# sumansamui/CMOOP_Audio_Processing

Hardware: AMD Instinct MI355X
Metric: candidate-net evals/hour (pop=40, GSC-v2) (higher is better)
Workload: dtype f32

## Files before the change

### cmoop_audio_processing_amd/_lib.py

```python
from __future__ import annotations

import ctypes as C
import os
import re
import subprocess
import threading

_HERE = os.path.dirname(os.path.abspath(__file__))
CSRC = os.path.join(_HERE, "csrc")
LIB_PATH = os.environ.get("CMOOP_LIB_PATH") or os.path.join(CSRC, "libcmoop_hip.so")
HEADER = os.path.join(os.path.dirname(_HERE), "include", "cmoop.h")

_lock = threading.Lock()
_lib = None


class CmoopError(RuntimeError):
    pass


class Config(C.Structure):
    _fields_ = [(n, C.c_int32) for n in (
        "variant", "classes", "epochs", "batch", "patience", "early_stop", "restore_best", "acc_readout",
        "fpr_variant", "shuffle", "eval_batch", "n_slots", "profile_every", "gemm_mode")] + \
# ... 355 lines not shown

def plan_convs(gene, variant, T, F):
    g, n, cap = (C.c_int32 * 6)(*gene), C.c_int32(), 16
    rows = (C.c_int32 * (7 * cap))()
    check(lib().cmoop_plan_convs(g, C.c_int32(variant), C.c_int32(T), C.c_int32(F), rows, C.c_int32(cap), C.byref(n)))
    assert n.value <= cap
    return [tuple(rows[7 * i:7 * i + 7]) for i in range(n.value)]


def plan_dwconvs(gene, variant, T, F):
    g, n, cap = (C.c_int32 * 6)(*gene), C.c_int32(), 16
    rows = (C.c_int32 * (4 * cap))()
    check(lib().cmoop_plan_dwconvs(g, C.c_int32(variant), C.c_int32(T), C.c_int32(F), rows, C.c_int32(cap), C.byref(n)))
    assert n.value <= cap
    return [tuple(rows[4 * i:4 * i + 4]) for i in range(n.value)]


def dwconv_wgrad_slices(B, H, W, Cn, KS):
    out = C.c_int32()
    check(lib().cmoop_dwconv_wgrad_slices(B, H, W, Cn, KS, C.byref(out)))
    return int(out.value)


def net_launch_plan(gene, config, T, F, B, train):
    g, buf = (C.c_int32 * 6)(*gene), C.create_string_buffer(8192)
    check(lib().cmoop_net_launch_plan(g, C.byref(config), C.c_int32(T), C.c_int32(F), C.c_int32(B), C.c_int32(int(train)), buf,
                                      C.c_int32(8192)))
    return [k for k in buf.value.decode().split(";") if k]


def profile_entries():
    L, cnt, out = lib(), C.c_int32(), []
    check(L.cmoop_profile_count(C.byref(cnt)))
    for i in range(cnt.value):
        name, n, ms, fl = C.create_string_buffer(160), C.c_int64(), C.c_double(), C.c_double()
        check(L.cmoop_profile_entry(i, name, 160, C.byref(n), C.byref(ms), C.byref(fl)))
        out.append((name.value.decode(), int(n.value), float(ms.value), float(fl.value)))
    return out


def profile_variants():
    L, cnt, out = lib(), C.c_int32(), []
    check(L.cmoop_profile_variant_count(C.byref(cnt)))
    for i in range(cnt.value):
        name = C.create_string_buffer(200)
        check(L.cmoop_profile_variant(i, name, 200))
# ... 13 lines not shown
```

### cmoop_audio_processing_amd/csrc/api.hip

```cpp
#include "../../include/cmoop.h"
#include "net.h"

#include <cstddef>
#include <cstring>
#include <memory>
#include <mutex>
#include <vector>

using namespace cmoop;

static thread_local std::string g_err;
static thread_local std::string g_last_kernels;

template <class F>
static int guard(F&& f) {
    try {
        f();
        return 0;
    } catch (const std::exception& e) {
        g_err = e.what();
        return 1;
    } catch (...) {
        g_err = "unknown error";
        return 2;
// ... 1298 lines not shown
        CMOOP_REQUIRE(out, "dwconv_wgrad_slices: NULL output");
        *out = dwconv_wgrad_slices(B, H, W, C, KS);
    });
}

int cmoop_net_launch_plan(const int32_t gene[6], const cmoop_config* cfg, int32_t T, int32_t F, int32_t B, int32_t train, char* buf,
                          int32_t cap) {
    return guard([&] {
        CMOOP_REQUIRE(gene && buf && cap > 0 && T >= 1 && F >= 1, "net_launch_plan: bad arguments");
        const NetConfig c = to_cfg(cfg);
        const std::string v = plan_net(gene, c, T, F).launch_plan(c.batch, std::max(c.batch, c.eval_batch), B, train != 0);
        CMOOP_REQUIRE((int)v.size() < cap, "net_launch_plan: buffer too small");
        std::memcpy(buf, v.c_str(), v.size() + 1);
    });
}

int cmoop_halo_tile_check(int32_t B, int32_t H, int32_t W, int32_t Cin, int32_t Cout, int32_t KS, int32_t* rows_bound,
                          int32_t* rows_needed, int32_t* rows_stageable) {
    return guard([&] {
        CMOOP_REQUIRE(rows_bound && rows_needed && rows_stageable && B >= 1 && H >= 1 && W >= 1 && Cin >= 16 && Cout >= 1 && KS >= 1, "bad conv shape");
        int b = 0, n = 0, c = 0;
        halo_rows_bound_and_need(conv_geometry(B, H, W, Cin, Cout, KS, 1), &b, &n, &c);
        *rows_bound = b; *rows_needed = n; *rows_stageable = c;
    });
}

int cmoop_wgrad_slices(int32_t B, int32_t H, int32_t W, int32_t Cin, int32_t Cout, int32_t KS, int32_t stride, int32_t* out) {
    return guard([&] {
        CMOOP_REQUIRE(out && B >= 1 && H >= 1 && W >= 1 && Cin >= 1 && Cout >= 1 && KS >= 1 && stride >= 1, "bad conv shape");
        *out = wgrad_slices(conv_geometry(B, H, W, Cin, Cout, KS, stride));
    });
}

int cmoop_calculate_fpr(const int32_t* y_true, const int32_t* y_pred, int64_t n, int32_t classes, int32_t fpr_variant,
                        double* out) {
    return guard([&] {
        CMOOP_REQUIRE(classes >= 1 && classes <= 4096, "bad class count");
        std::vector<int64_t> cm((size_t)classes * classes, 0);
        for (int64_t i = 0; i < n; ++i) {
            const int a = fpr_variant == CMOOP_FPR_V1_QUIRK ? 0 : y_true[i];
            const int b = y_pred[i];
            if (a >= 0 && a < classes && b >= 0 && b < classes) cm[(size_t)a * classes + b] += 1;
        }
        *out = fpr_from_confusion(cm.data(), classes, fpr_variant == CMOOP_FPR_V3 ? 2 : 0);
    });
}
// ... 759 lines not shown
        CMOOP_HIP(hipStreamSynchronize(s));
    });
}

int cmoop_conv_bwd_trainer(const float* x, const float* w, const float* dy, float* dx, float* dw, float* db, int32_t B, int32_t H,
                           int32_t W, int32_t Cin, int32_t Cout, int32_t KS, int32_t stride, int32_t mask_relu) {
    return guard([&] {
        g_last_kernels.clear();
        hipStream_t s = lib_stream();
        Scratch m(s);
        const ConvLayer L{H, W, Cin, Cout, KS, stride};
        RecordingHook hook(&g_last_kernels);
        const size_t NK = L.flip_floats();
        ConvBuffers buf;
        buf.slab_floats = L.slab_floats_at(B);
        buf.slabs = m.floats(buf.slab_floats);
        float* dwb = m.floats(NK + Cout);
        buf.tab_rows = L.table_rows(B);
        buf.tab = m.rowtab(L.geometry(B), buf.tab_rows);
        L.wgrad(x, dy, dwb, dwb + NK, B, buf, GEMM_DEFAULT, s, &hook);
        CMOOP_HIP(hipMemcpyAsync(dw, dwb, NK * 4, hipMemcpyDeviceToDevice, s));
        CMOOP_HIP(hipMemcpyAsync(db, dwb + NK, (size_t)Cout * 4, hipMemcpyDeviceToDevice, s));
        if (dx) {
            int accumulate = 0;
            if (stride != 1) {
                CMOOP_HIP(hipMemsetAsync(dx, 0, (size_t)B * H * W * Cin * 4, s));
                accumulate = 1;
            }
            if (L.mfma_dgrad()) {
                buf.wd = m.floats(NK);
                launch_flip_transpose(w, buf.wd, Cout, KS, KS, Cin, s);
                buf.tab_d_rows = L.dgrad_table_rows(B);
                buf.tab_d = m.rowtab(L.dgrad_geom(B), buf.tab_d_rows);
                buf.splitk_floats = igemm_splitk_workspace(L.dgrad_geom(B));
                buf.splitk = m.floats(buf.splitk_floats);
            }
            L.dgrad(dy, w, dx, B, mask_relu ? x : nullptr, 1.f, accumulate, L.mfma_dgrad(), buf, GEMM_DEFAULT, s, &hook);
        }
        CMOOP_HIP(hipStreamSynchronize(s));
    });
}

int cmoop_last_kernels(char* buf, int32_t cap) {
    return guard([&] {
        CMOOP_REQUIRE(buf && cap > 0, "last_kernels: no buffer");
        std::snprintf(buf, cap, "%s", g_last_kernels.c_str());
    });
}

int cmoop_conv_time(int32_t mode, const float* x, const float* w, const float* bias, float* y, int32_t B, int32_t H,
                    int32_t W, int32_t Cin, int32_t Cout, int32_t KS, int32_t iters, double* avg_ms) {
    return guard([&] {
        hipStream_t s = lib_stream();
        Scratch m(s);
        const ConvLayer L{H, W, Cin, Cout, KS, 1};
        const ConvGeom g = L.geometry(B), gd = L.dgrad_geom(B);
        float *wd = nullptr, *wg = nullptr;
        GemmEpilogue e;
        const int S = wgrad_slices(g);
        if (mode == 0) e.bias = bias;
// ... 287 lines not shown
```

### cmoop_audio_processing_amd/csrc/gemm.hip

```cpp
#include "kernels.h"
#include <hip/hip_ext.h>
#include <cstdlib>
#include <mutex>
#include <string>
#include <type_traits>

namespace cmoop {

typedef __bf16 bf16x8 __attribute__((ext_vector_type(8)));
typedef unsigned u32x4 __attribute__((ext_vector_type(4)));

typedef __bf16 bf16x2 __attribute__((ext_vector_type(2)));

template <int NP>
__device__ __forceinline__ void split_pair(const float x, const float y, unsigned (&w)[NP]) {
    if constexpr (NP == 1) {
        w[0] = __builtin_bit_cast(unsigned, __builtin_convertvector((f32x2){x, y}, bf16x2));
    } else {
        const unsigned ux = __float_as_uint(x), uy = __float_as_uint(y);
        w[0] = __builtin_amdgcn_perm(uy, ux, 0x07060302u);
        const float rx = x - __uint_as_float(ux & 0xFFFF0000u), ry = y - __uint_as_float(uy & 0xFFFF0000u);
        const unsigned vx = __float_as_uint(rx), vy = __float_as_uint(ry);
        w[1] = __builtin_amdgcn_perm(vy, vx, 0x07060302u);
        const float sx = rx - __uint_as_float(vx & 0xFFFF0000u), sy = ry - __uint_as_float(vy & 0xFFFF0000u);
// ... 7 lines not shown
int gemm_mode_default() {
    static const int v = [] {
        const char* e = std::getenv("CMOOP_GEMM_MODE");
        if (!e) return (int)GEMM_FP32;
        const std::string m(e);
        return m == "bf16x3" ? (int)GEMM_BF16X3 : (m == "bf16" ? (int)GEMM_BF16 : (int)GEMM_FP32);
    }();
    return v;
}
static int resolve_mode(int mode) {
    const int m = mode >= 0 ? mode : gemm_mode_default();
    return (m == GEMM_BF16X3 || m == GEMM_BF16) ? m : GEMM_FP32;
}

struct GeomDev {
    int B, H, W, Cin, OH, OW, Cout, KH, KW, stride, pad_t, pad_l;
    int M, K, cshift, OHW;
    uint32_t ohw_magic, ohw_shift, ow_magic, ow_shift;
    int rcp_kw;
    const float* zeros;
};
struct EpiDev {
    int bal_L, bal_segmax;
    float* stats;
    const float* bias;
    const float* mask;
    float mask_scale;
    int relu, accumulate, out_stride, OHf, OWf, dropout;
    uint32_t drop_prefix, drop_thr;
    float drop_scale;
};

static double par_scale() {
    static const double v = [] {
        const char* e = std::getenv("CMOOP_PAR_SCALE");
        const double x = e ? std::atof(e) : 1.0;
        return x > 0.01 && x <= 4.0 ? x : 1.0;
    }();
    return v;
}

__device__ __forceinline__ int fastdiv(int n, uint32_t magic, uint32_t shift) {
    return (int)((__umulhi((uint32_t)n, magic) + (uint32_t)n) >> shift);
}

static const float* zero_page() {
// ... 575 lines not shown
                red[((wave / WN) * BN + c) * 2 + 1] = csq[ct];
            }
        }
        __syncthreads();
        if (t < BN && n0 + t < N) {
            float a = 0.f, b = 0.f;
#pragma unroll
            for (int w = 0; w < WM; ++w) { a += red[(w * BN + t) * 2]; b += red[(w * BN + t) * 2 + 1]; }
            e.stats[((size_t)mtile * 2) * N + n0 + t] = a;
            e.stats[((size_t)mtile * 2 + 1) * N + n0 + t] = b;
        }
    }
    }
}

struct HaloDev {
    int WP, rows_max, VH;
    uint32_t wp_magic, wp_shift, vh_magic, vh_shift;
};
__host__ __device__ constexpr int halo_nst(int bm) { return bm == 256 ? 11 : 9; }
static bool halo_geometry(const ConvGeom& cg, HaloDev* hd, size_t* lds_bytes);
static size_t halo_balanced_slab_floats(const ConvGeom& cg, int* L_out);

template <int KS, int BM, int BN, int WM, bool BAL = false>
__global__ __launch_bounds__(256, 2) void halo_fwd_kernel(const float* __restrict__ X, const float* __restrict__ Wt,
                                                          float* __restrict__ Y, GeomDev g, EpiDev e, HaloDev h,
                                                          float* __restrict__ slab) {
    constexpr int WN = 4 / WM, RT = BM / WM / 16, CT = BN / WN / 16, R = KS / 2, T = KS * KS;
    constexpr int PITCH = 24;
    constexpr int NST = halo_nst(BM);
    static_assert(RT >= 1 && CT >= 1, "tile too small for the wave layout");
    extern __shared__ __attribute__((aligned(16))) float halo[];

    const int t = threadIdx.x;
    const int ncc = g.Cin >> 4;
    const int upt = ncc * KS;
    int u = 0, uend = 1;
    if constexpr (BAL) {
        const int U = ((g.M + BM - 1) / BM) * ((g.Cout + BN - 1) / BN) * upt;
        u = blockIdx.x * e.bal_L;
        uend = min(U, u + e.bal_L);
    }
    while (u < uend) {
    int mtile, ntile, c_lo = 0, c_hi = upt;
    float* pslab = nullptr;
    if constexpr (BAL) {
        const int nt = (g.Cout + BN - 1) / BN;
        const int t0 = u / upt;
        c_lo = u - t0 * upt;
        c_hi = min(upt, c_lo + (uend - u));
        mtile = t0 / nt; ntile = t0 - mtile * nt;
        const int seg = c_lo == 0 ? 0 : (int)blockIdx.x - (t0 * upt) / e.bal_L;
        pslab = slab + ((size_t)t0 * e.bal_segmax + seg) * (BM * BN);
        u += c_hi - c_lo;
        __syncthreads();
    } else {
        u = uend;
        mtile = blockIdx.x;
        const int nwg = gridDim.x, xcd = mtile & 7, idx = mtile >> 3;
        const int qn = nwg >> 3, rn = nwg & 7;
        mtile = (xcd < rn ? xcd * (qn + 1) : rn * (qn + 1) + (xcd - rn) * qn) + idx;
        ntile = blockIdx.y;
    }
    const int m0 = mtile * BM, n0 = ntile * BN;
    const int wave = t >> 6, lane = t & 63, lr = lane & 15, q = lane >> 4;
    const int wrow = (wave / WN) * (BM / WM), wcol = (wave % WN) * (BN / WN);

    auto vrow = [&](int m, int& x) {
        const int b = fastdiv(m, g.ohw_magic, g.ohw_shift), r = m - b * g.OHW;
        const int y = fastdiv(r, g.ow_magic, g.ow_shift);
        x = r - y * g.OW;
        return b * h.VH + y;
    };
    int xdummy;
    const int vbase = vrow(m0, xdummy);
    const int vlast = vrow(min(m0 + BM, g.M) - 1, xdummy);
    const int items = (vlast - vbase + 1 + 2 * R) * h.WP * 4;

    const __amdgpu_buffer_rsrc_t xr = __builtin_amdgcn_make_buffer_rsrc(
        const_cast<float*>(X), 0, (int)((uint32_t)g.B * g.H * g.W << g.cshift) * 4, 0x00020000);
// ... 82 lines not shown
#pragma unroll
                for (int j = 0; j < 4; ++j)
#pragma unroll
                    for (int rt = 0; rt < RT; ++rt)
#pragma unroll
                        for (int ct = 0; ct < CT; ++ct)
                            acc[rt][ct] = __builtin_amdgcn_mfma_f32_16x16x4f32(ac[rt][j], bc[ct][j], acc[rt][ct], 0, 0, 0);
                __builtin_amdgcn_s_setprio(0);
#pragma unroll
                for (int ct = 0; ct < CT; ++ct) bc[ct] = bn[ct];
                if (kx + 1 < KS || (!last_unit && !new_cc)) {
#pragma unroll
                    for (int rt = 0; rt < RT; ++rt) ac[rt] = an[rt];
                } else if (!last_unit) {
                    __syncthreads();
                    stage_store();
                    __syncthreads();
#pragma unroll
                    for (int rt = 0; rt < RT; ++rt) ac[rt] = *reinterpret_cast<const f32x4*>(a_ptr[rt]);
                }
            }
            ky = nky; cc = ncc2;
        }
#pragma unroll
        for (int rt = 0; rt < RT; ++rt)
#pragma unroll
            for (int r = 0; r < 4; ++r)
#pragma unroll
                for (int ct = 0; ct < CT; ++ct)
                    pslab[(wrow + rt * 16 + q * 4 + r) * BN + wcol + ct * 16 + lr] = acc[rt][ct][r];
        continue;
    } else {
    f32x4 ac[RT], bc[CT];
    stage_load(0);
    load_b(0, 0, bc);
    stage_store();
    __syncthreads();
#pragma unroll
    for (int rt = 0; rt < RT; ++rt) ac[rt] = *reinterpret_cast<const f32x4*>(a_ptr[rt]);

    for (int cc = 0; cc < ncc; ++cc) {
        const bool more = cc + 1 < ncc;
#pragma unroll
        for (int tap = 0; tap < T; ++tap) {
            f32x4 an[RT], bn[CT];
#pragma unroll
            for (int ct = 0; ct < CT; ++ct) bn[ct] = bc[ct];
            if (tap + 1 < T) {
                load_b(cc, tap + 1, bn);
                const int ky = (tap + 1) / KS, kx = (tap + 1) % KS;
#pragma unroll
                for (int rt = 0; rt < RT; ++rt)
                    an[rt] = *reinterpret_cast<const f32x4*>(a_ptr[rt] + ky * wp_f + kx * PITCH);
            } else if (more) {
// ... 7 lines not shown
                for (int rt = 0; rt < RT; ++rt)
#pragma unroll
                    for (int ct = 0; ct < CT; ++ct)
                        acc[rt][ct] = __builtin_amdgcn_mfma_f32_16x16x4f32(ac[rt][j], bc[ct][j], acc[rt][ct], 0, 0, 0);
            __builtin_amdgcn_s_setprio(0);
#pragma unroll
            for (int ct = 0; ct < CT; ++ct) bc[ct] = bn[ct];
            if (tap + 1 < T) {
#pragma unroll
                for (int rt = 0; rt < RT; ++rt) ac[rt] = an[rt];
            } else if (more) {
                __syncthreads();
                stage_store();
                __syncthreads();
#pragma unroll
                for (int rt = 0; rt < RT; ++rt) ac[rt] = *reinterpret_cast<const f32x4*>(a_ptr[rt]);
            }
        }
    }

    }

    const int N = g.Cout;
    float csum[CT], csq[CT], bias_v[CT];
#pragma unroll
    for (int ct = 0; ct < CT; ++ct) {
        csum[ct] = 0.f; csq[ct] = 0.f;
        const int col = n0 + wcol + ct * 16 + lr;
        bias_v[ct] = (e.bias && col < N) ? e.bias[col] : 0.f;
    }
    const bool whole = m0 + BM <= g.M && (N % BN) == 0;
    const uint32_t e_lane = (uint32_t)((m0 + wrow + q * 4) * N + n0 + wcol + lr) * 4u;
    const __amdgpu_buffer_rsrc_t yrs = __builtin_amdgcn_make_buffer_rsrc(Y, 0, g.M * N * 4, 0x00020000);
    if (whole && !e.dropout && !e.mask && !e.accumulate) {
        auto store_all = [&](auto relu_c, auto stats_c) {
#pragma unroll
            for (int rt = 0; rt < RT; ++rt)
#pragma unroll
                for (int r = 0; r < 4; ++r) {
                    const int soff = (rt * 16 + r) * N * 4;
#pragma unroll
                    for (int ct = 0; ct < CT; ++ct) {
                        float v = acc[rt][ct][r] + bias_v[ct];
                        if constexpr (decltype(relu_c)::value) v = fmaxf(v, 0.f);
                        __builtin_amdgcn_raw_buffer_store_b32(__float_as_uint(v), yrs, (int)(e_lane + ct * 64), soff, 0);
                        if constexpr (decltype(stats_c)::value) { csum[ct] += v; csq[ct] += v * v; }
                    }
                }
        };
        using T1 = std::integral_constant<bool, true>;
        using T0 = std::integral_constant<bool, false>;
        if (e.relu) { if (e.stats) store_all(T1{}, T1{}); else store_all(T1{}, T0{}); }
        else        { if (e.stats) store_all(T0{}, T1{}); else store_all(T0{}, T0{}); }
    } else if (whole && e.mask && !e.dropout && !e.relu && !e.bias && !e.stats) {
        const __amdgpu_buffer_rsrc_t mrs = __builtin_amdgcn_make_buffer_rsrc(const_cast<float*>(e.mask), 0, g.M * N * 4, 0x00020000);
#pragma unroll
        for (int rt = 0; rt < RT; ++rt) {
            float mk[4][CT], old[4][CT];
#pragma unroll
            for (int r = 0; r < 4; ++r)
#pragma unroll
                for (int ct = 0; ct < CT; ++ct) {
                    const int soff = (rt * 16 + r) * N * 4;
                    mk[r][ct] = __uint_as_float(__builtin_amdgcn_raw_buffer_load_b32(mrs, (int)(e_lane + ct * 64), soff, 0));
                    old[r][ct] = e.accumulate ? __uint_as_float(__builtin_amdgcn_raw_buffer_load_b32(yrs, (int)(e_lane + ct * 64), soff, 0)) : 0.f;
                }
#pragma unroll
            for (int r = 0; r < 4; ++r)
#pragma unroll
                for (int ct = 0; ct < CT; ++ct) {
                    const int soff = (rt * 16 + r) * N * 4;
                    float v = (mk[r][ct] > 0.f) ? acc[rt][ct][r] * e.mask_scale : 0.f;
                    if (e.accumulate) v += old[r][ct];
                    __builtin_amdgcn_raw_buffer_store_b32(__float_as_uint(v), yrs, (int)(e_lane + ct * 64), soff, 0);
                }
        }
    } else {
// ... 4 lines not shown
            const int row = m0 + wrow + rt * 16 + q * 4 + r;
            if (row >= g.M) continue;
            const size_t rbase = (size_t)row * N;
#pragma unroll
            for (int ct = 0; ct < CT; ++ct) {
                const int col = n0 + wcol + ct * 16 + lr;
                if (col >= N) continue;
                float v = acc[rt][ct][r] + bias_v[ct];
                if (e.relu) v = fmaxf(v, 0.f);
                const size_t off = rbase + col;
                if (e.dropout) {
                    uint32_t u24 = fmix32(e.drop_prefix ^ (uint32_t)((size_t)row * N + col)) >> 8;
                    v = (u24 >= e.drop_thr) ? v * e.drop_scale : 0.f;
                }
                if (e.mask) v = (e.mask[off] > 0.f) ? v * e.mask_scale : 0.f;
                if (e.accumulate) v += Y[off];
                Y[off] = v;
                csum[ct] += v;
                csq[ct] += v * v;
            }
        }
    }
    }
    if (e.stats) {
        __syncthreads();
        float* red = halo;
#pragma unroll
        for (int ct = 0; ct < CT; ++ct) {
            csum[ct] += __shfl_xor(csum[ct], 16, 64);
            csq[ct] += __shfl_xor(csq[ct], 16, 64);
            csum[ct] += __shfl_xor(csum[ct], 32, 64);
            csq[ct] += __shfl_xor(csq[ct], 32, 64);
            if (q == 0) {
                const int c = wcol + ct * 16 + lr;
                red[((wave / WN) * BN + c) * 2] = csum[ct];
                red[((wave / WN) * BN + c) * 2 + 1] = csq[ct];
            }
        }
        __syncthreads();
        if (t < BN && n0 + t < N) {
            float a = 0.f, b = 0.f;
#pragma unroll
            for (int w = 0; w < WM; ++w) { a += red[(w * BN + t) * 2]; b += red[(w * BN + t) * 2 + 1]; }
            e.stats[((size_t)mtile * 2) * N + n0 + t] = a;
            e.stats[((size_t)mtile * 2 + 1) * N + n0 + t] = b;
        }
    }
    }
}

struct BalDev { int bm, bn, nt, chunks, L, segmax; };

template <int VEC>
__global__ __launch_bounds__(256) void splitk_combine_kernel(const float* __restrict__ P, float* __restrict__ Y, GeomDev g,
                                                             EpiDev e, int splits, BalDev bal) {
    const int N = g.Cout;
    const size_t total = (size_t)g.M * N;
    for (size_t i = ((size_t)blockIdx.x * 256 + threadIdx.x) * VEC; i < total; i += (size_t)gridDim.x * 256 * VEC) {
        const int row = (int)(i / N), col = (int)(i - (size_t)row * N);
        float v[VEC];
#pragma unroll
        for (int j = 0; j < VEC; ++j) v[j] = 0.f;
        if (bal.L > 0) {
            const int mt = row / bal.bm, ntl = col / bal.bn;
            const int tile = mt * bal.nt + ntl;
            const int first = (tile * bal.chunks) / bal.L;
            const int nseg = ((tile + 1) * bal.chunks + bal.L - 1) / bal.L - first;
            const float* src = P + (size_t)tile * bal.segmax * (bal.bm * bal.bn) + (size_t)(row - mt * bal.bm) * bal.bn + (col - ntl * bal.bn);
            for (int z = 0; z < nseg; ++z) {
                if constexpr (VEC == 4) {
                    const f32x4 p = *reinterpret_cast<const f32x4*>(src + (size_t)z * (bal.bm * bal.bn));
                    v[0] += p[0]; v[1] += p[1]; v[2] += p[2]; v[3] += p[3];
                } else {
                    v[0] += src[(size_t)z * (bal.bm * bal.bn)];
                }
            }
        } else
        for (int z = 0; z < splits; ++z) {
            if constexpr (VEC == 4) {
                const f32x4 p = *reinterpret_cast<const f32x4*>(P + (size_t)z * total + i);
                v[0] += p[0]; v[1] += p[1]; v[2] += p[2]; v[3] += p[3];
            } else {
                v[0] += P[(size_t)z * total + i];
            }
        }
        size_t off = i;
        if (e.out_stride != 1) {
            int b = fastdiv(row, g.ohw_magic, g.ohw_shift), rr = row - b * g.OHW;
            int oh = fastdiv(rr, g.ow_magic, g.ow_shift), ow = rr - oh * g.OW;
            off = ((size_t)(b * e.OHf + oh * e.out_stride) * e.OWf + ow * e.out_stride) * N + col;
        }
#pragma unroll
        for (int j = 0; j < VEC; ++j) {
            float x = v[j];
            if (e.bias) x += e.bias[col + j];
            if (e.relu) x = fmaxf(x, 0.f);
            if (e.dropout) {
                uint32_t u24 = fmix32(e.drop_prefix ^ (uint32_t)(i + j)) >> 8;
                x = (u24 >= e.drop_thr) ? x * e.drop_scale : 0.f;
            }
            if (e.mask) x = (e.mask[off + j] > 0.f) ? x * e.mask_scale : 0.f;
            if (e.accumulate) x += Y[off + j];
            v[j] = x;
        }
        if constexpr (VEC == 4) *reinterpret_cast<f32x4*>(Y + off) = f32x4{v[0], v[1], v[2], v[3]};
        else Y[off] = v[0];
    }
// ... 110 lines not shown
    *bm = 64; *bn = bn_small;
}

size_t igemm_splitk_workspace(const ConvGeom& g) {
    const int M = g.M(), N = g.Cout;
    const int bn_big = N > 64 ? 128 : (N <= 16 ? 16 : (N <= 32 ? 32 : 64));
    const long blocks = (long)cdiv(M, 128) * cdiv(N, bn_big);
    if (blocks >= 384) return 0;
    const int sp = std::min(32, cdiv(1024, (int)blocks));
    return std::max(std::max((size_t)sp * M * N, balanced_slab_floats(M, N, g.K(), g.Cin % 32 == 0 ? 32 : 16, bn_big, nullptr)),
                    halo_balanced_slab_floats(g, nullptr));
}

static size_t halo_balanced_slab_floats(const ConvGeom& cg, int* L_out) {
    static const bool on = [] { const char* v = std::getenv("CMOOP_HALO_BAL"); return !(v && v[0] == '0'); }();
    if (!on || cg.Cout % 64 != 0 || !halo_geometry(cg, nullptr, nullptr)) return 0;
    const long tiles = (long)cdiv(cg.M(), 128) * (cg.Cout / 64);
    const int upt = (cg.Cin / 16) * cg.KH;
    const long units = tiles * upt;
    if (tiles >= 1024 || units < 512l * 2 * cg.KH) return 0;
    const int L = (int)((units + 511) / 512);
    if (L_out) *L_out = L;
    return (size_t)tiles * (cdiv(upt, L) + 1) * 128 * 64;
}

struct FwdChoice {
    int mode, bm, bn, splits, balanced_wgs, flags;
    bool bk32_tile, use_dma, stats, halo;
    int ks, halo_L;
    int code() const { return mode * 100000000 + bm * 100000 + bn * 100 + (halo ? ks + (halo_L > 0 ? 50 : 0) : (bk32_tile ? 32 : 16)); }
};

static inline int halo_bm(int cout) { return cout >= 64 ? 128 : 256; }
static bool halo_geometry(const ConvGeom& cg, HaloDev* hd, size_t* lds_bytes) {
    const int ks = cg.KH, R = ks / 2;
    if (cg.KH != cg.KW || (ks != 3 && ks != 5) || cg.stride != 1 || cg.OH != cg.H || cg.OW != cg.W) return false;
    if (cg.pad_t != R || cg.pad_l != R || cg.Cin % 16 != 0) return false;
    if (cg.Cout % 64 != 0 && cg.Cout != 32 && cg.Cout != 16) return false;
    const int bm = halo_bm(cg.Cout);
    const int wp = (cg.W + ks - 1 + 7) / 8 * 8;
    const int span = (bm - 2 + cg.W) / cg.W + 1 + ((bm - 1) / (cg.H * cg.W) + 1) * R;
    const int rows = span + 2 * R;
    if (rows * wp * 4 > halo_nst(bm) * 256) return false;
    const size_t lds = (size_t)rows * wp * 24 * sizeof(float);
    if (lds > 64 * 1024) return false;
    if (hd) {
// ... 47 lines not shown
        c.bm = halo_bm(cg.Cout);
        c.bn = std::min(cg.Cout, 64);
    } else if (halo_env && (c.mode == GEMM_FP32 || c.mode == GEMM_FP32_DMA) && c.bm == 128 && (c.splits > 1 || c.balanced_wgs) && ep.out_stride == 1) {
        int L = 0;
        const size_t need = halo_balanced_slab_floats(cg, &L);
        if (need > 0 && need <= ws_floats) {
            c.halo = true; c.halo_L = L; c.mode = GEMM_FP32_HALO; c.use_dma = false; c.stats = false;
            c.bm = 128; c.bn = 64; c.splits = 1; c.balanced_wgs = 512;
        }
    }
    c.flags = (c.splits > 1 ? GEMM_FLAG_SPLITK : 0) | (c.stats ? GEMM_FLAG_STATS : 0) | (c.balanced_wgs ? GEMM_FLAG_BALANCED : 0) |
              ((!c.halo && have_rowtab && (cg.Cin % bk) == 0 && cg.KH * cg.KW <= 32) ? GEMM_FLAG_ROWTAB : 0);
    return c;
}

int igemm_fwd_plan(const ConvGeom& g, const GemmEpilogue& ep, size_t ws_floats, bool want_stats, bool have_rowtab, int* flags_out) {
    igemm_check_range(g);
    CMOOP_REQUIRE(ilog2_exact(g.Cin) >= 4, "implicit GEMM needs C_in a power of two >= 16");
    const FwdChoice c = choose_fwd(g, ep, ws_floats, want_stats, have_rowtab);
    if (flags_out) *flags_out = c.flags;
    return c.code();
}

int launch_igemm_fwd(const float* X, const float* Wt, float* Y, const ConvGeom& cg, const GemmEpilogue& ep,
                     hipStream_t s, const GemmTiming* tm, float* splitk_ws, size_t splitk_ws_floats, int* stats_blocks,
                     const void* rowtab_v, int tab_rows, int* flags_out) {
    if (stats_blocks) *stats_blocks = 0;
    if (flags_out) *flags_out = 0;
    const uint2* rowtab = static_cast<const uint2*>(rowtab_v);
    GeomDev g = to_dev(cg);
    if (g.M == 0) return 0;
    EpiDev e;
    e.bias = ep.bias; e.mask = ep.mask; e.mask_scale = ep.mask_scale; e.relu = ep.relu;
    e.accumulate = ep.accumulate; e.out_stride = ep.out_stride; e.OHf = ep.OHf; e.OWf = ep.OWf;
    e.dropout = ep.dropout; e.drop_prefix = ep.drop_prefix; e.drop_thr = ep.drop_thr; e.drop_scale = ep.drop_scale;
    if (e.out_stride > 1)
        CMOOP_REQUIRE((int64_t)g.B * e.OHf * e.OWf * g.Cout < (1ll << 29), "scattered output too large");
    const FwdChoice ch = choose_fwd(cg, ep, splitk_ws ? splitk_ws_floats : 0, ep.stats != nullptr && stats_blocks != nullptr, rowtab != nullptr);
    const int mode = ch.mode == GEMM_FP32_DMA ? (int)GEMM_FP32 : ch.mode;
    const int bm = ch.bm, bn = ch.bn, splits = ch.splits, balanced_wgs = ch.balanced_wgs;
    const bool bk32_tile = ch.bk32_tile, use_dma = ch.use_dma;
    e.bal_L = 0; e.bal_segmax = 0;
    e.stats = ch.stats ? ep.stats : nullptr;
    if (e.stats) *stats_blocks = cdiv(g.M, bm);
    if (flags_out) *flags_out = ch.flags;
    if (ch.halo) {
        HaloDev hd;
        size_t lds = 0;
        CMOOP_REQUIRE(halo_geometry(cg, &hd, &lds), "halo kernel chosen for a geometry it does not accept");
        dim3 grid(cdiv(g.M, bm), cdiv(g.Cout, bn));
        BalDev bal{bm, bn, cdiv(g.Cout, bn), (cg.Cin / 16) * cg.KH, ch.halo_L, 0};
        if (ch.halo_L > 0) {
            bal.segmax = cdiv(bal.chunks, bal.L) + 1;
            e.bal_L = bal.L; e.bal_segmax = bal.segmax;
            const long units = (long)grid.x * grid.y * bal.chunks;
            grid = dim3((unsigned)((units + bal.L - 1) / bal.L), 1, 1);
            lds = std::max(lds, (size_t)55 * 1024);
        }
        static const int occ_env = [] { const char* v = std::getenv("CMOOP_HALO_OCC"); const int o = v ? std::atoi(v) : 0; return o == 2 || o == 3 ? o : 0; }();
        lds = halo_lds_for_occupancy(lds, (long)grid.x * grid.y, occ_env);
        auto run = [&](auto kernel) { launch_timed(kernel, grid, lds, s, tm, X, Wt, Y, g, e, hd, splitk_ws); };
#define CMOOP_HALO_KS(KS_)                                                                     \
        do {                                                                                   \
            if (ch.halo_L > 0) run(halo_fwd_kernel<KS_, 128, 64, 2, true>);                    \
            else if (bn == 64) run(halo_fwd_kernel<KS_, 128, 64, 2, false>);                   \
            else if (bn == 32) run(halo_fwd_kernel<KS_, 256, 32, 4, false>);                   \
            else run(halo_fwd_kernel<KS_, 256, 16, 4, false>);                                 \
        } while (0)
        if (cg.KH == 5) CMOOP_HALO_KS(5); else CMOOP_HALO_KS(3);
#undef CMOOP_HALO_KS
        CMOOP_HIP(hipGetLastError());
        if (ch.halo_L > 0) {
            const size_t total = (size_t)g.M * g.Cout;
            const unsigned gridc = (unsigned)std::min<size_t>((total / 4 + 255) / 256, 4096);
            hipLaunchKernelGGL(splitk_combine_kernel<4>, dim3(gridc), dim3(256), 0, s, splitk_ws, Y, g, e, 2, bal);
            CMOOP_HIP(hipGetLastError());
        }
        return ch.code();
    }
#define CMOOP_FWD(BM_, BN_, WM_)                                                              \
    do {                                                                                      \
        if (mode == GEMM_BF16X3) launch_fwd_t<BM_, BN_, 32, WM_, GEMM_BF16X3>(X, Wt, Y, g, e, s, tm, splitk_ws, splits, balanced_wgs, rowtab, tab_rows);   \
        else if (mode == GEMM_BF16) launch_fwd_t<BM_, BN_, 32, WM_, GEMM_BF16>(X, Wt, Y, g, e, s, tm, splitk_ws, splits, balanced_wgs, rowtab, tab_rows);  \
        else if (use_dma && BM_ == 128 && BN_ == 32) launch_fwd_t<BM_, 32, 32, WM_, GEMM_FP32_DMA>(X, Wt, Y, g, e, s, tm, splitk_ws, splits, balanced_wgs, rowtab, tab_rows);   \
        else if (bk32_tile) launch_fwd_t<BM_, BN_, 32, WM_>(X, Wt, Y, g, e, s, tm, splitk_ws, splits, balanced_wgs, rowtab, tab_rows);   \
        else launch_fwd_t<BM_, BN_, 16, WM_>(X, Wt, Y, g, e, s, tm, splitk_ws, splits, 0, rowtab, tab_rows);        \
    } while (0)
    if (bm == 128) {
        if (bn == 128) CMOOP_FWD(128, 128, 2);
        else if (bn == 64) CMOOP_FWD(128, 64, 4);
        else if (bn == 32) CMOOP_FWD(128, 32, 4);
        else CMOOP_FWD(128, 16, 4);
    } else {
        if (bn == 64) CMOOP_FWD(64, 64, 2);
        else if (bn == 32) CMOOP_FWD(64, 32, 4);
        else CMOOP_FWD(64, 16, 4);
// ... 796 lines not shown
```

### cmoop_audio_processing_amd/csrc/kernels.h

```cpp
#pragma once
#include "common.h"
#include <string>
#include <vector>

namespace cmoop {

struct ConvGeom {
    int B, H, W, Cin;
    int OH, OW, Cout;
    int KH, KW, stride;
    int pad_t, pad_l;
    int M() const { return B * OH * OW; }
    int K() const { return KH * KW * Cin; }
};
inline ConvGeom conv_geometry(int B, int H, int W, int Cin, int Cout, int KS, int stride) {
    ConvGeom g;
    g.B = B; g.H = H; g.W = W; g.Cin = Cin; g.Cout = Cout; g.KH = g.KW = KS; g.stride = stride;
    g.OH = (H + stride - 1) / stride; g.OW = (W + stride - 1) / stride;
    const int th = (g.OH - 1) * stride + KS - H, tw = (g.OW - 1) * stride + KS - W;
    g.pad_t = (th > 0 ? th : 0) / 2; g.pad_l = (tw > 0 ? tw : 0) / 2;
    return g;
}

enum GemmMode { GEMM_DEFAULT = -1, GEMM_FP32 = 0, GEMM_FP32_DMA = 1 , GEMM_BF16X3 = 2, GEMM_BF16 = 3,
// ... 8 lines not shown
    float mask_scale = 1.f;
    int accumulate = 0;
    int out_stride = 1;
    int OHf = 0, OWf = 0;
    int dropout = 0;
    uint32_t drop_prefix = 0, drop_thr = 0;
    float drop_scale = 1.f;
    float* stats = nullptr;
};

struct GemmTiming {
    hipEvent_t start = nullptr, stop = nullptr;
    bool ext = true;
};
enum GemmFlags { GEMM_FLAG_SPLITK = 1, GEMM_FLAG_STATS = 2, GEMM_FLAG_ROWTAB = 4, GEMM_FLAG_BALANCED = 8, GEMM_FLAG_SLABS = 16 };
int launch_igemm_fwd(const float* X, const float* Wt, float* Y, const ConvGeom& g,
                     const GemmEpilogue& e, hipStream_t s, const GemmTiming* tm = nullptr,
                     float* splitk_ws = nullptr, size_t splitk_ws_floats = 0, int* stats_blocks = nullptr,
                     const void* rowtab = nullptr, int tab_rows = 0, int* flags_out = nullptr);
size_t igemm_splitk_workspace(const ConvGeom& g);
int igemm_fwd_plan(const ConvGeom& g, const GemmEpilogue& e, size_t ws_floats, bool want_stats, bool have_rowtab, int* flags_out);
int igemm_wgrad_plan(const ConvGeom& g, int S, int mode, bool have_rowtab, int* flags_out);
void halo_rows_bound_and_need(const ConvGeom& g, int* bound, int* need, int* items_cap);
void igemm_check_range(const ConvGeom& g);
std::string gemm_kernel_name(int cls, int code);

int wgrad_slices(const ConvGeom& g);
int launch_igemm_wgrad(const float* X, const float* dY, float* P, const ConvGeom& g, int S, hipStream_t s,
                       const GemmTiming* tm = nullptr, float* Pbias = nullptr, size_t slab_stride = 0,
                       int mode = GEMM_DEFAULT, const void* rowtab = nullptr, int tab_rows = 0, int* flags_out = nullptr);
int rowtab_rows(const ConvGeom& g);
void launch_build_rowtab(const ConvGeom& g, void* tab, hipStream_t s);
void launch_reduce_slices(const float* P, float* out, int S, int64_t n, hipStream_t s, int64_t stride = 0);
void launch_flip_transpose(const float* W, float* Wd, int Cout, int KH, int KW, int Cin, hipStream_t s);
struct FlipEntry { int64_t w_off, wd_off; int Cout, KH, KW, Cin; };
void launch_flip_transpose_all(const float* params, float* wd_all, const FlipEntry* table_dev, int layers, int64_t max_elems,
                               hipStream_t s);

struct StepState {
    long long row0;
    unsigned step;
    unsigned iter;
};
void launch_step_advance(StepState* st, int batch, hipStream_t s);
struct BatchRows {
    const int32_t* idx = nullptr;
// ... 404 lines not shown
```

### include/cmoop.h

```cpp
#ifndef CMOOP_H
#define CMOOP_H

#include <stdint.h>

#ifdef __cplusplus
extern "C" {
#endif

#define CMOOP_ABI_VERSION 3

#define CMOOP_VARIANT_A 0
#define CMOOP_VARIANT_B 1
#define CMOOP_VARIANT_A_DS 2
#define CMOOP_VARIANT_B_DS 3

#define CMOOP_FPR_V1 0
#define CMOOP_FPR_V1_QUIRK 1
#define CMOOP_FPR_V3 2

#define CMOOP_GEMM_DEFAULT 0
#define CMOOP_GEMM_FP32 1
#define CMOOP_GEMM_BF16X3 2
#define CMOOP_GEMM_BF16 3

// ... 278 lines not shown
                             const cmoop_optim* optim, const cmoop_ema* ema, const cmoop_opoint* op, const cmoop_quant* q,
                             const cmoop_prune* pr, const cmoop_actquant* aq, const cmoop_dataset* ds, const int32_t* genes ,
                             const uint32_t* seeds , int32_t n, cmoop_next_fn next, void* ctx, double* acc, double* size_mb,
                             double* fpr, int32_t* epochs_run, double* val_loss, double* seconds, int32_t* evaluated,
                             double* opoint , double* quant ,
                             double* prune );

int cmoop_plan_check(const int32_t gene[6], int32_t variant, int32_t T, int32_t F, int32_t batch);

int cmoop_conv_launch_plan(int32_t op, int32_t B, int32_t H, int32_t W, int32_t Cin, int32_t Cout, int32_t KS, int32_t stride,
                           int32_t want_stats, char* name, int32_t name_cap);

int cmoop_plan_convs(const int32_t gene[6], int32_t variant, int32_t T, int32_t F, int32_t* layers , int32_t cap,
                     int32_t* count);

int cmoop_plan_dwconvs(const int32_t gene[6], int32_t variant, int32_t T, int32_t F, int32_t* layers , int32_t cap,
                       int32_t* count);

int cmoop_net_launch_plan(const int32_t gene[6], const cmoop_config* cfg, int32_t T, int32_t F, int32_t B, int32_t train,
                          char* buf, int32_t cap);

int cmoop_halo_tile_check(int32_t B, int32_t H, int32_t W, int32_t Cin, int32_t Cout, int32_t KS, int32_t* rows_bound,
                          int32_t* rows_needed, int32_t* rows_stageable);

int cmoop_wgrad_slices(int32_t B, int32_t H, int32_t W, int32_t Cin, int32_t Cout, int32_t KS, int32_t stride, int32_t* out);

int cmoop_dwconv_wgrad_slices(int32_t B, int32_t H, int32_t W, int32_t C, int32_t KS, int32_t* out);

int cmoop_calculate_fpr(const int32_t* y_true, const int32_t* y_pred, int64_t n, int32_t classes, int32_t fpr_variant,
                        double* out);

int cmoop_logmel(const float* wav_dev , int64_t n_clips, int32_t n_samples,
                 float* out_dev );
typedef struct cmoop_frontend_config {
    int32_t sr, n_fft, win, hop, n_mels;
    int32_t scale;
    int32_t db_ref_max;
    float fmin, fmax, log_eps, db_amin, top_db;
} cmoop_frontend_config;
int cmoop_frontend_config_default(cmoop_frontend_config* c);
int cmoop_frontend_check(const cmoop_frontend_config* c);
int cmoop_frontend_frames(const cmoop_frontend_config* c, int32_t n_samples, int32_t* T);
int cmoop_frontend_mel_basis(const cmoop_frontend_config* c, float* out_host);
int cmoop_logmel_ex(const cmoop_frontend_config* c, const float* wav_dev , int64_t n_clips,
                    int32_t n_samples, float* out_dev );
int cmoop_logmel_ex_time(const cmoop_frontend_config* c, const float* wav_dev, int64_t n_clips, int32_t n_samples, float* out_dev,
// ... 174 lines not shown
```

Baseline: 440.9.

## Give each balanced halo workgroup one whole tile plus a stream-K share

Restructures the stream-K balanced halo forward conv so that each of the G workgroups first computes one complete output tile through the normal epilogue, then splits the remaining tiles' K-units evenly. Only the split tiles go through the slab workspace and the combine kernel. This cuts slab writes and combine traffic for most of the output. It is gated on an env switch (on by default) and on workspace fitting, and the combine kernel gains a tile-indexed path. A host-side partition checker is added for validation, and the dgrad test entry gains an accumulate flag.

```diff
diff --git a/cmoop_audio_processing_amd/_lib.py b/cmoop_audio_processing_amd/_lib.py
--- a/cmoop_audio_processing_amd/_lib.py
+++ b/cmoop_audio_processing_amd/_lib.py
@@ -401,6 +401,22 @@
     return int(out.value)
 
 
+HALO_BAL_FIELDS = ("T", "upt", "L", "G", "s", "whole", "slab_floats", "workgroups", "most_units", "finished_in_kernel", "cut_tiles",
+                   "slab_pieces", "units_not_owned_once", "slab_faults", "combine_elements", "is_bal")
+
+
+def halo_bal_partition_check(B, H, W, Cin, Cout, KS, ws_floats=-1, whole=-1, pieces_cap=0):
+    out, n = (C.c_int64 * 16)(), C.c_int32()
+    rows = (C.c_int32 * (5 * pieces_cap))() if pieces_cap > 0 else None
+    check(lib().cmoop_halo_bal_partition_check(C.c_int32(B), C.c_int32(H), C.c_int32(W), C.c_int32(Cin), C.c_int32(Cout), C.c_int32(KS),
+                                               C.c_int64(ws_floats), C.c_int32(whole), out, rows, C.c_int32(pieces_cap), C.byref(n)))
+    res = dict(zip(HALO_BAL_FIELDS, (int(v) for v in out)))
+    if rows is not None:
+        assert n.value <= pieces_cap, "pieces_cap too small"
+        res["pieces"] = [tuple(rows[5 * i:5 * i + 5]) for i in range(n.value)]
+    return res
+
+
 def net_launch_plan(gene, config, T, F, B, train):
     g, buf = (C.c_int32 * 6)(*gene), C.create_string_buffer(8192)
     check(lib().cmoop_net_launch_plan(g, C.byref(config), C.c_int32(T), C.c_int32(F), C.c_int32(B), C.c_int32(int(train)), buf,
diff --git a/cmoop_audio_processing_amd/csrc/api.hip b/cmoop_audio_processing_amd/csrc/api.hip
--- a/cmoop_audio_processing_amd/csrc/api.hip
+++ b/cmoop_audio_processing_amd/csrc/api.hip
@@ -1344,6 +1344,20 @@
         int b = 0, n = 0, c = 0;
         halo_rows_bound_and_need(conv_geometry(B, H, W, Cin, Cout, KS, 1), &b, &n, &c);
         *rows_bound = b; *rows_needed = n; *rows_stageable = c;
+    });
+}
+
+int cmoop_halo_bal_partition_check(int32_t B, int32_t H, int32_t W, int32_t Cin, int32_t Cout, int32_t KS, int64_t ws_floats,
+                                   int32_t whole, int64_t out[16], int32_t* pieces, int32_t pieces_cap, int32_t* n_pieces) {
+    return guard([&] {
+        CMOOP_REQUIRE(out && B >= 1 && H >= 1 && W >= 1 && Cin >= 16 && Cout >= 1 && KS >= 1 && pieces_cap >= 0 && (pieces || pieces_cap == 0),
+                      "halo_bal_partition_check: bad arguments");
+        const ConvGeom g = conv_geometry(B, H, W, Cin, Cout, KS, 1);
+        igemm_check_range(g);
+        CMOOP_REQUIRE((Cin & (Cin - 1)) == 0, "implicit GEMM needs C_in a power of two >= 16");
+        const size_t ws = ws_floats < 0 ? igemm_splitk_workspace(g) : (size_t)ws_floats;
+        const int64_t n = halo_bal_partition_walk(g, ws, whole < 0 ? -1 : (whole != 0), out, pieces, pieces_cap);
+        if (n_pieces) *n_pieces = (int32_t)n;
     });
 }
 
@@ -2149,8 +2163,8 @@
         CMOOP_HIP(hipMemcpyAsync(dw, dwb, NK * 4, hipMemcpyDeviceToDevice, s));
         CMOOP_HIP(hipMemcpyAsync(db, dwb + NK, (size_t)Cout * 4, hipMemcpyDeviceToDevice, s));
         if (dx) {
-            int accumulate = 0;
-            if (stride != 1) {
+            int accumulate = (mask_relu & 2) ? 1 : 0;
+            if (stride != 1 && !accumulate) {
                 CMOOP_HIP(hipMemsetAsync(dx, 0, (size_t)B * H * W * Cin * 4, s));
                 accumulate = 1;
             }
@@ -2162,7 +2176,7 @@
                 buf.splitk_floats = igemm_splitk_workspace(L.dgrad_geom(B));
                 buf.splitk = m.floats(buf.splitk_floats);
             }
-            L.dgrad(dy, w, dx, B, mask_relu ? x : nullptr, 1.f, accumulate, L.mfma_dgrad(), buf, GEMM_DEFAULT, s, &hook);
+            L.dgrad(dy, w, dx, B, (mask_relu & 1) ? x : nullptr, 1.f, accumulate, L.mfma_dgrad(), buf, GEMM_DEFAULT, s, &hook);
         }
         CMOOP_HIP(hipStreamSynchronize(s));
     });
diff --git a/cmoop_audio_processing_amd/csrc/gemm.hip b/cmoop_audio_processing_amd/csrc/gemm.hip
--- a/cmoop_audio_processing_amd/csrc/gemm.hip
+++ b/cmoop_audio_processing_amd/csrc/gemm.hip
@@ -53,6 +53,7 @@
 };
 struct EpiDev {
     int bal_L, bal_segmax;
+    int bal_G, bal_s;
     float* stats;
     const float* bias;
     const float* mask;
@@ -674,6 +675,32 @@
 static bool halo_geometry(const ConvGeom& cg, HaloDev* hd, size_t* lds_bytes);
 static size_t halo_balanced_slab_floats(const ConvGeom& cg, int* L_out);
 
+struct BalWalk { int u, uend, own; };
+__host__ __device__ inline BalWalk bal_walk_begin(int w, int T, int upt, int L, int G_whole, int s) {
+    BalWalk k;
+    const int per = G_whole > 0 ? s : L, end = (G_whole > 0 ? T - G_whole : T) * upt;
+    k.own = G_whole > 0;
+    k.u = w * per < end ? w * per : end;
+    k.uend = k.u + per < end ? k.u + per : end;
+    return k;
+}
+__host__ __device__ inline bool bal_walk_more(const BalWalk& k) { return k.own || k.u < k.uend; }
+__host__ __device__ inline void bal_walk_next(BalWalk& k, int w, int upt, int L, int segmax, int G_whole, int s, int& tile,
+                                              int& c_lo, int& c_hi, int& slot) {
+    if (k.own) { k.own = 0; tile = w; c_lo = 0; c_hi = upt; slot = -1; return; }
+    const int per = G_whole > 0 ? s : L;
+    const int t0 = k.u / upt;
+    c_lo = k.u - t0 * upt;
+    c_hi = c_lo + (k.uend - k.u) < upt ? c_lo + (k.uend - k.u) : upt;
+    const int seg = c_lo == 0 ? 0 : w - (t0 * upt) / per;
+    tile = G_whole + t0;
+    slot = (G_whole > 0 && c_lo == 0 && c_hi == upt) ? -1 : t0 * segmax + seg;
+    k.u += c_hi - c_lo;
+}
+__host__ __device__ inline int bal_tile_pieces(int t0, int upt, int per) {
+    return ((t0 + 1) * upt + per - 1) / per - (t0 * upt) / per;
+}
+
 template <int KS, int BM, int BN, int WM, bool BAL = false>
 __global__ __launch_bounds__(256, 2) void halo_fwd_kernel(const float* __restrict__ X, const float* __restrict__ Wt,
                                                           float* __restrict__ Y, GeomDev g, EpiDev e, HaloDev h,
@@ -687,27 +714,21 @@
     const int t = threadIdx.x;
     const int ncc = g.Cin >> 4;
     const int upt = ncc * KS;
-    int u = 0, uend = 1;
-    if constexpr (BAL) {
-        const int U = ((g.M + BM - 1) / BM) * ((g.Cout + BN - 1) / BN) * upt;
-        u = blockIdx.x * e.bal_L;
-        uend = min(U, u + e.bal_L);
-    }
-    while (u < uend) {
+    BalWalk bw{0, 1, 0};
+    if constexpr (BAL)
+        bw = bal_walk_begin((int)blockIdx.x, ((g.M + BM - 1) / BM) * ((g.Cout + BN - 1) / BN), upt, e.bal_L, e.bal_G, e.bal_s);
+    while (bal_walk_more(bw)) {
     int mtile, ntile, c_lo = 0, c_hi = upt;
     float* pslab = nullptr;
     if constexpr (BAL) {
         const int nt = (g.Cout + BN - 1) / BN;
-        const int t0 = u / upt;
-        c_lo = u - t0 * upt;
-        c_hi = min(upt, c_lo + (uend - u));
+        int t0, slot;
+        bal_walk_next(bw, (int)blockIdx.x, upt, e.bal_L, e.bal_segmax, e.bal_G, e.bal_s, t0, c_lo, c_hi, slot);
         mtile = t0 / nt; ntile = t0 - mtile * nt;
-        const int seg = c_lo == 0 ? 0 : (int)blockIdx.x - (t0 * upt) / e.bal_L;
-        pslab = slab + ((size_t)t0 * e.bal_segmax + seg) * (BM * BN);
-        u += c_hi - c_lo;
+        if (slot >= 0) pslab = slab + (size_t)slot * (BM * BN);
         __syncthreads();
     } else {
-        u = uend;
+        bw.u = bw.uend;
         mtile = blockIdx.x;
         const int nwg = gridDim.x, xcd = mtile & 7, idx = mtile >> 3;
         const int qn = nwg >> 3, rn = nwg & 7;
@@ -836,14 +857,16 @@
             }
             ky = nky; cc = ncc2;
         }
-#pragma unroll
-        for (int rt = 0; rt < RT; ++rt)
-#pragma unroll
-            for (int r = 0; r < 4; ++r)
-#pragma unroll
-                for (int ct = 0; ct < CT; ++ct)
-                    pslab[(wrow + rt * 16 + q * 4 + r) * BN + wcol + ct * 16 + lr] = acc[rt][ct][r];
-        continue;
+        if (pslab) {
+#pragma unroll
+            for (int rt = 0; rt < RT; ++rt)
+#pragma unroll
+                for (int r = 0; r < 4; ++r)
+#pragma unroll
+                    for (int ct = 0; ct < CT; ++ct)
+                        pslab[(wrow + rt * 16 + q * 4 + r) * BN + wcol + ct * 16 + lr] = acc[rt][ct][r];
+            continue;
+        }
     } else {
     f32x4 ac[RT], bc[CT];
     stage_load(0);
@@ -897,6 +920,7 @@
     }
 
     const int N = g.Cout;
+    float* const stats = BAL ? nullptr : e.stats;
     float csum[CT], csq[CT], bias_v[CT];
 #pragma unroll
     for (int ct = 0; ct < CT; ++ct) {
@@ -925,9 +949,9 @@
         };
         using T1 = std::integral_constant<bool, true>;
         using T0 = std::integral_constant<bool, false>;
-        if (e.relu) { if (e.stats) store_all(T1{}, T1{}); else store_all(T1{}, T0{}); }
-        else        { if (e.stats) store_all(T0{}, T1{}); else store_all(T0{}, T0{}); }
-    } else if (whole && e.mask && !e.dropout && !e.relu && !e.bias && !e.stats) {
+        if (e.relu) { if (stats) store_all(T1{}, T1{}); else store_all(T1{}, T0{}); }
+        else        { if (stats) store_all(T0{}, T1{}); else store_all(T0{}, T0{}); }
+    } else if (whole && e.mask && !e.dropout && !e.relu && !e.bias && !stats) {
         const __amdgpu_buffer_rsrc_t mrs = __builtin_amdgcn_make_buffer_rsrc(const_cast<float*>(e.mask), 0, g.M * N * 4, 0x00020000);
 #pragma unroll
         for (int rt = 0; rt < RT; ++rt) {
@@ -978,7 +1002,7 @@
         }
     }
     }
-    if (e.stats) {
+    if (stats) {
         __syncthreads();
         float* red = halo;
 #pragma unroll
@@ -998,25 +1022,63 @@
             float a = 0.f, b = 0.f;
 #pragma unroll
             for (int w = 0; w < WM; ++w) { a += red[(w * BN + t) * 2]; b += red[(w * BN + t) * 2 + 1]; }
-            e.stats[((size_t)mtile * 2) * N + n0 + t] = a;
-            e.stats[((size_t)mtile * 2 + 1) * N + n0 + t] = b;
-        }
-    }
-    }
-}
-
-struct BalDev { int bm, bn, nt, chunks, L, segmax; };
+            stats[((size_t)mtile * 2) * N + n0 + t] = a;
+            stats[((size_t)mtile * 2 + 1) * N + n0 + t] = b;
+        }
+    }
+    }
+}
+
+struct BalDev { int bm, bn, nt, chunks, L, segmax, G, T; };
 
 template <int VEC>
 __global__ __launch_bounds__(256) void splitk_combine_kernel(const float* __restrict__ P, float* __restrict__ Y, GeomDev g,
                                                              EpiDev e, int splits, BalDev bal) {
     const int N = g.Cout;
     const size_t total = (size_t)g.M * N;
-    for (size_t i = ((size_t)blockIdx.x * 256 + threadIdx.x) * VEC; i < total; i += (size_t)gridDim.x * 256 * VEC) {
-        const int row = (int)(i / N), col = (int)(i - (size_t)row * N);
+    const size_t count = bal.G > 0 ? (size_t)(bal.T - bal.G) * (bal.bm * bal.bn) : total;
+    for (size_t k = ((size_t)blockIdx.x * 256 + threadIdx.x) * VEC; k < count; k += (size_t)gridDim.x * 256 * VEC) {
+        size_t i = k;
+        int row, col;
         float v[VEC];
 #pragma unroll
         for (int j = 0; j < VEC; ++j) v[j] = 0.f;
+        if (bal.G > 0) {
+            const int t0 = (int)(k / (size_t)(bal.bm * bal.bn)), in_tile = (int)(k - (size_t)t0 * (bal.bm * bal.bn));
+            const int tile = bal.G + t0, mt = tile / bal.nt, ntl = tile - mt * bal.nt;
+            row = mt * bal.bm + in_tile / bal.bn;
+            col = ntl * bal.bn + in_tile % bal.bn;
+            const int nseg = bal_tile_pieces(t0, bal.chunks, bal.L);
+            if (row >= g.M || nseg == 1) continue;
+            i = (size_t)row * N + col;
+            const float* src = P + (size_t)t0 * bal.segmax * (bal.bm * bal.bn) + in_tile;
+            int z = 0;
+            for (; z + 8 <= nseg; z += 8) {
+                float p[8][VEC];
+#pragma unroll
+                for (int b = 0; b < 8; ++b) {
+                    if constexpr (VEC == 4) {
+                        const f32x4 q = *reinterpret_cast<const f32x4*>(src + (size_t)(z + b) * (bal.bm * bal.bn));
+                        p[b][0] = q[0]; p[b][1] = q[1]; p[b][2] = q[2]; p[b][3] = q[3];
+                    } else {
+                        p[b][0] = src[(size_t)(z + b) * (bal.bm * bal.bn)];
+                    }
+                }
+#pragma unroll
+                for (int b = 0; b < 8; ++b)
+#pragma unroll
+                    for (int j = 0; j < VEC; ++j) v[j] += p[b][j];
+            }
+            for (; z < nseg; ++z) {
+                if constexpr (VEC == 4) {
+                    const f32x4 p = *reinterpret_cast<const f32x4*>(src + (size_t)z * (bal.bm * bal.bn));
+                    v[0] += p[0]; v[1] += p[1]; v[2] += p[2]; v[3] += p[3];
+                } else {
+                    v[0] += src[(size_t)z * (bal.bm * bal.bn)];
+                }
+            }
+        } else {
+        row = (int)(i / N); col = (int)(i - (size_t)row * N);
         if (bal.L > 0) {
             const int mt = row / bal.bm, ntl = col / bal.bn;
             const int tile = mt * bal.nt + ntl;
@@ -1039,6 +1101,7 @@
             } else {
                 v[0] += P[(size_t)z * total + i];
             }
+        }
         }
         size_t off = i;
         if (e.out_stride != 1) {
@@ -1195,6 +1258,30 @@
     const int L = (int)((units + 511) / 512);
     if (L_out) *L_out = L;
     return (size_t)tiles * (cdiv(upt, L) + 1) * 128 * 64;
+}
+
+struct HaloBalPart {
+    int T, upt, L, G, s, segmax;
+    bool whole;
+    size_t slab_floats;
+};
+static HaloBalPart halo_bal_partition(const ConvGeom& cg, int L, size_t ws_floats, int whole_switch) {
+    static const bool env_on = [] { const char* v = std::getenv("CMOOP_HALO_BAL_WHOLE"); return !(v && v[0] == '0'); }();
+    HaloBalPart p;
+    p.T = cdiv(cg.M(), 128) * (cg.Cout / 64);
+    p.upt = (cg.Cin / 16) * cg.KH;
+    p.L = L;
+    p.G = cdiv(p.T * p.upt, L);
+    p.s = L - p.upt;
+    p.whole = false;
+    p.segmax = cdiv(p.upt, L) + 1;
+    p.slab_floats = (size_t)p.T * p.segmax * 128 * 64;
+    if ((whole_switch < 0 ? env_on : whole_switch != 0) && p.T >= p.G) {
+        const int segmax = p.s > 0 ? cdiv(p.upt, p.s) + 1 : 0;
+        const size_t need = (size_t)(p.T - p.G) * segmax * 128 * 64;
+        if (need <= ws_floats) { p.whole = true; p.segmax = segmax; p.slab_floats = need; }
+    }
+    return p;
 }
 
 struct FwdChoice {
@@ -1288,6 +1375,52 @@
     return c.code();
 }
 
+int64_t halo_bal_partition_walk(const ConvGeom& cg, size_t ws_floats, int whole_switch, int64_t out[16], int32_t* pieces, int cap) {
+    for (int i = 0; i < 16; ++i) out[i] = 0;
+    const FwdChoice ch = choose_fwd(cg, GemmEpilogue(), ws_floats, false, true);
+    if (!(ch.halo && ch.halo_L > 0)) return 0;
+    const HaloBalPart p = halo_bal_partition(cg, ch.halo_L, ws_floats, whole_switch);
+    const int Gw = p.whole ? p.G : 0, first_cut = Gw, per = p.whole ? p.s : p.L;
+    const int64_t slots = (int64_t)(p.slab_floats / (128 * 64));
+    std::vector<int> owned((size_t)p.T * p.upt, 0), in_kernel(p.T, 0), in_slab(p.T, 0);
+    std::vector<char> slot_used((size_t)slots, 0);
+    int64_t most = 0, npieces = 0, faults = 0;
+    for (int w = 0; w < p.G; ++w) {
+        BalWalk k = bal_walk_begin(w, p.T, p.upt, p.L, Gw, p.s);
+        int64_t mine = 0;
+        while (bal_walk_more(k)) {
+            int tile, c_lo, c_hi, slot;
+            bal_walk_next(k, w, p.upt, p.L, p.segmax, Gw, p.s, tile, c_lo, c_hi, slot);
+            if (pieces && npieces < cap) {
+                const int32_t row[5] = {w, tile, c_lo, c_hi, slot};
+                for (int i = 0; i < 5; ++i) pieces[5 * npieces + i] = row[i];
+            }
+            ++npieces;
+            if (tile < 0 || tile >= p.T || c_lo < 0 || c_hi > p.upt || c_lo >= c_hi) { ++faults; break; }
+            for (int c = c_lo; c < c_hi; ++c) ++owned[(size_t)tile * p.upt + c];
+            mine += c_hi - c_lo;
+            if (slot < 0) { ++in_kernel[tile]; faults += !(c_lo == 0 && c_hi == p.upt); continue; }
+            const int seg = slot - (tile - first_cut) * p.segmax;
+            faults += seg != in_slab[tile] || seg >= p.segmax;
+            ++in_slab[tile];
+            if (slot >= slots || slot_used[slot]) ++faults; else slot_used[slot] = 1;
+        }
+        most = std::max(most, mine);
+    }
+    int64_t finished = 0, cut = 0, slab_pieces = 0, bad_units = 0;
+    for (int v : owned) bad_units += v != 1;
+    for (int t = 0; t < p.T; ++t) {
+        finished += in_kernel[t] > 0; cut += in_slab[t] > 0; slab_pieces += in_slab[t];
+        const int nseg = t >= first_cut ? bal_tile_pieces(t - first_cut, p.upt, per) : 0;
+        const bool combined = t >= first_cut && !(p.whole && nseg == 1);
+        faults += combined ? (in_slab[t] != nseg || in_kernel[t] != 0) : (in_slab[t] != 0 || in_kernel[t] != 1);
+    }
+    out[0] = p.T; out[1] = p.upt; out[2] = p.L; out[3] = p.G; out[4] = p.s; out[5] = p.whole; out[6] = (int64_t)p.slab_floats;
+    out[7] = p.G; out[8] = most; out[9] = finished; out[10] = cut; out[11] = slab_pieces; out[12] = bad_units; out[13] = faults;
+    out[14] = p.whole ? (int64_t)(p.T - p.G) * 128 * 64 : (int64_t)cg.M() * cg.Cout; out[15] = 1;
+    return npieces;
+}
+
 int launch_igemm_fwd(const float* X, const float* Wt, float* Y, const ConvGeom& cg, const GemmEpilogue& ep,
                      hipStream_t s, const GemmTiming* tm, float* splitk_ws, size_t splitk_ws_floats, int* stats_blocks,
                      const void* rowtab_v, int tab_rows, int* flags_out) {
@@ -1306,7 +1439,7 @@
     const int mode = ch.mode == GEMM_FP32_DMA ? (int)GEMM_FP32 : ch.mode;
     const int bm = ch.bm, bn = ch.bn, splits = ch.splits, balanced_wgs = ch.balanced_wgs;
     const bool bk32_tile = ch.bk32_tile, use_dma = ch.use_dma;
-    e.bal_L = 0; e.bal_segmax = 0;
+    e.bal_L = 0; e.bal_segmax = 0; e.bal_G = 0; e.bal_s = 0;
     e.stats = ch.stats ? ep.stats : nullptr;
     if (e.stats) *stats_blocks = cdiv(g.M, bm);
     if (flags_out) *flags_out = ch.flags;
@@ -1316,11 +1449,13 @@
         CMOOP_REQUIRE(halo_geometry(cg, &hd, &lds), "halo kernel chosen for a geometry it does not accept");
         dim3 grid(cdiv(g.M, bm), cdiv(g.Cout, bn));
         BalDev bal{bm, bn, cdiv(g.Cout, bn), (cg.Cin / 16) * cg.KH, ch.halo_L, 0};
+        HaloBalPart part{};
         if (ch.halo_L > 0) {
-            bal.segmax = cdiv(bal.chunks, bal.L) + 1;
-            e.bal_L = bal.L; e.bal_segmax = bal.segmax;
-            const long units = (long)grid.x * grid.y * bal.chunks;
-            grid = dim3((unsigned)((units + bal.L - 1) / bal.L), 1, 1);
+            part = halo_bal_partition(cg, ch.halo_L, splitk_ws_floats, -1);
+            bal.segmax = part.segmax;
+            e.bal_L = part.L; e.bal_segmax = part.segmax;
+            if (part.whole) { e.bal_G = part.G; e.bal_s = part.s; bal.L = part.s; bal.G = part.G; bal.T = part.T; }
+            grid = dim3((unsigned)part.G, 1, 1);
             lds = std::max(lds, (size_t)55 * 1024);
         }
         static const int occ_env = [] { const char* v = std::getenv("CMOOP_HALO_OCC"); const int o = v ? std::atoi(v) : 0; return o == 2 || o == 3 ? o : 0; }();
@@ -1336,8 +1471,8 @@
         if (cg.KH == 5) CMOOP_HALO_KS(5); else CMOOP_HALO_KS(3);
 #undef CMOOP_HALO_KS
         CMOOP_HIP(hipGetLastError());
-        if (ch.halo_L > 0) {
-            const size_t total = (size_t)g.M * g.Cout;
+        const size_t total = part.whole ? (size_t)(part.T - part.G) * (bm * bn) : (size_t)g.M * g.Cout;
+        if (ch.halo_L > 0 && total > 0) {
             const unsigned gridc = (unsigned)std::min<size_t>((total / 4 + 255) / 256, 4096);
             hipLaunchKernelGGL(splitk_combine_kernel<4>, dim3(gridc), dim3(256), 0, s, splitk_ws, Y, g, e, 2, bal);
             CMOOP_HIP(hipGetLastError());
diff --git a/cmoop_audio_processing_amd/csrc/kernels.h b/cmoop_audio_processing_amd/csrc/kernels.h
--- a/cmoop_audio_processing_amd/csrc/kernels.h
+++ b/cmoop_audio_processing_amd/csrc/kernels.h
@@ -54,6 +54,7 @@
 int igemm_fwd_plan(const ConvGeom& g, const GemmEpilogue& e, size_t ws_floats, bool want_stats, bool have_rowtab, int* flags_out);
 int igemm_wgrad_plan(const ConvGeom& g, int S, int mode, bool have_rowtab, int* flags_out);
 void halo_rows_bound_and_need(const ConvGeom& g, int* bound, int* need, int* items_cap);
+int64_t halo_bal_partition_walk(const ConvGeom& g, size_t ws_floats, int whole_switch, int64_t out[16], int32_t* pieces, int cap);
 void igemm_check_range(const ConvGeom& g);
 std::string gemm_kernel_name(int cls, int code);
 
diff --git a/include/cmoop.h b/include/cmoop.h
--- a/include/cmoop.h
+++ b/include/cmoop.h
@@ -324,6 +324,10 @@
 
 int cmoop_halo_tile_check(int32_t B, int32_t H, int32_t W, int32_t Cin, int32_t Cout, int32_t KS, int32_t* rows_bound,
                           int32_t* rows_needed, int32_t* rows_stageable);
+
+int cmoop_halo_bal_partition_check(int32_t B, int32_t H, int32_t W, int32_t Cin, int32_t Cout, int32_t KS, int64_t ws_floats,
+                                   int32_t whole, int64_t out[16], int32_t* pieces , int32_t pieces_cap,
+                                   int32_t* n_pieces);
 
 int cmoop_wgrad_slices(int32_t B, int32_t H, int32_t W, int32_t Cin, int32_t Cout, int32_t KS, int32_t stride, int32_t* out);
 
```

Result: no change. 441.6 (median of 6 runs) (+0.2%).
